# automl/CARL

Measured on AMD Instinct MI355X. Metric: env-steps/sec (whole node) at 65k parallel contexts, 1/2/4/8 MI355X, higher is better.
Workload: dtype f32

## Files before the change

### carl_amd/csrc/carl_amd.hip

```cpp
#include <hip/hip_runtime.h>

#include <cmath>
#include <cstdarg>
#include <cstdio>
#include <cstdlib>
#include <cstring>
#include <map>
#include <mutex>
#include <utility>

#include "../../include/carl_amd.h"
#include "classic_control.hip.h"
#include "context_kernels.hip.h"
#include "engine_kernels.hip.h"
#include "host_common.hpp"

namespace carl_host {

thread_local char g_err[512] = "";

int fail(int code, const char* fmt, ...) {
  va_list ap;
  va_start(ap, fmt);
  vsnprintf(g_err, sizeof g_err, fmt, ap);
// ... 124 lines not shown
}

}

namespace {

using carl_host::check_launch;
using carl_host::fail;
using carl_host::kInfo;
using carl_host::validate_batch;
using carl_host::with_classic_family;

int validate_io(const carl_batch_t* b, const carl_step_io_t* io, const char* who) {
  if (io == nullptr) return fail(CARL_ERR_INVALID_ARGUMENT, "%s: io is NULL", who);
  if (!io->action || !io->obs || !io->reward || !io->terminated || !io->truncated)
    return fail(CARL_ERR_INVALID_ARGUMENT, "%s: a required io pointer is NULL", who);
  const bool discrete = kInfo[b->family].action_is_discrete != 0;
  if (discrete && io->action_dtype != CARL_ACTION_I32 && io->action_dtype != CARL_ACTION_I64 &&
      io->action_dtype != CARL_ACTION_U8)
    return fail(CARL_ERR_INVALID_ARGUMENT, "%s: discrete family needs int32/int64 (carl_rollout: or uint8) actions", who);
  if (io->action_dtype == CARL_ACTION_U8 && (reinterpret_cast<uintptr_t>(io->action) & 3) != 0)
    return fail(CARL_ERR_INVALID_ARGUMENT, "%s: uint8 actions must be 4-byte aligned", who);
  const bool half = io->action_dtype == CARL_ACTION_F16 || io->action_dtype == CARL_ACTION_BF16;
  if (!discrete && io->action_dtype != CARL_ACTION_F32 && !half)
    return fail(CARL_ERR_INVALID_ARGUMENT, "%s: continuous family needs float32 (carl_rollout: or float16 / bfloat16) actions", who);
  if (half && (reinterpret_cast<uintptr_t>(io->action) & 7) != 0)
    return fail(CARL_ERR_INVALID_ARGUMENT, "%s: float16 / bfloat16 actions must be 8-byte aligned", who);
  if (io->row_pitch != 0 && io->row_pitch < b->n_lanes)
    return fail(CARL_ERR_INVALID_ARGUMENT, "%s: io.row_pitch %d < n_lanes %d (0 = dense rows)", who, io->row_pitch, b->n_lanes);
  return 0;
}

template <class Fam>
bool use_lds_ctx(const carl_batch_t* b) {
  const size_t bytes = (size_t)Fam::F * b->n_contexts * sizeof(float);
  return bytes <= 32 * 1024 && (int64_t)b->n_contexts * 8 <= (int64_t)b->n_lanes;
}

int row_pitch_of(const carl_batch_t* b, const carl_step_io_t* io) { return io->row_pitch > 0 ? io->row_pitch : b->n_lanes; }

struct RolloutPlan {
  int variant = CARL_ROLLOUT_STAGED;
  bool lean = false;
  bool unsupported = false;
  int ak = 0;
  bool plain = false, ldsctx = false, moves = false, fin = false, ar = false, deep = false;
  size_t lds_bytes = 0;
};

template <class Fam>
RolloutPlan plan_rollout(const carl_batch_t* b, const carl_step_io_t* io) {
  static_assert(carl::predraw_of<Fam>::value, "the staged kernels below are instantiated for predrawing families");
  RolloutPlan p;
  const int dt = io->action_dtype;
  p.ak = dt == CARL_ACTION_I64 ? 1 : dt == CARL_ACTION_U8 ? carl::kActU8 : dt == CARL_ACTION_F16 ? carl::kActF16
         : dt == CARL_ACTION_BF16 ? carl::kActBF16 : 0;
  const uintptr_t amask = p.ak == carl::kActU8 ? 3u : p.ak > carl::kActU8 ? 7u : 15u;
  if (b->flags & CARL_FLAG_ROLLOUT_DIRECT)
    p.variant = CARL_ROLLOUT_DIRECT_FLAG;
  else if (!carl_host::staged_rows(b, io, amask))
    p.variant = CARL_ROLLOUT_DIRECT_SHAPE;
  const bool keeps_context = b->selector == CARL_SEL_STATIC || b->selector == CARL_SEL_HOST;
  p.lean = p.variant == CARL_ROLLOUT_STAGED && keeps_context && b->fin_count == nullptr && io->final_obs == nullptr;
  p.unsupported = p.ak >= carl::kActU8 && !p.lean;
  if (p.variant != CARL_ROLLOUT_STAGED) return p;

  p.lds_bytes = carl::rollout_staged_lds_bytes<Fam>();
  const size_t table_bytes = (size_t)Fam::F * b->n_contexts * sizeof(float);
  const bool table_fits =
      use_lds_ctx<Fam>(b) && p.lds_bytes + table_bytes + carl::static_lds_bytes<Fam>() <= carl::kCuLdsBytes;
  if (p.lean) {
    p.plain = true;
    p.ar = carl::dense_done_of<Fam>::value && (b->flags & CARL_FLAG_AUTORESET);
    p.deep = p.ak == 0 && b->n_lanes < carl::deep_below_lanes_of<Fam>::value;
  } else if (carl::dense_done_of<Fam>::value && b->fin_count == nullptr) {
    p.plain = true;
    p.moves = !keeps_context;
    p.fin = io->final_obs != nullptr;
    p.ldsctx = p.moves && table_fits;
  } else {
    p.ldsctx = !keeps_context && table_fits;
  }
  if (p.ldsctx) p.lds_bytes += table_bytes;
  return p;
}

using staged_kern_t = void (*)(carl_batch_t, carl_step_io_t, int);

template <class Fam>
staged_kern_t staged_kernel(const RolloutPlan& p) {
#define CARL_STAGED(AK, PLAIN, LDSCTX, MOVES, FIN, AR, DEEP)                                                         \
  if (p.ak == AK && p.plain == PLAIN && p.ldsctx == LDSCTX && p.moves == MOVES && p.fin == FIN && p.ar == AR &&    \
      p.deep == DEEP)                                                                                              \
    return carl::rollout_staged_kernel<Fam, AK, bool(PLAIN), bool(LDSCTX), bool(MOVES), bool(FIN), bool(AR), bool(DEEP)>;
#define CARL_STAGED_01(...) CARL_STAGED(0, __VA_ARGS__) CARL_STAGED(1, __VA_ARGS__)
  constexpr bool dense = carl::dense_done_of<Fam>::value, deep = carl::deep_below_lanes_of<Fam>::value > 0;
  CARL_STAGED_01(    0,     0,    0,  0, 0,   0)
  CARL_STAGED_01(    0,     1,    0,  0, 0,   0)
  CARL_STAGED_01(    1,     0,    0,  0, 0,   0)
  if constexpr (std::is_same_v<typename Fam::Action, int>) {
    CARL_STAGED(carl::kActU8, 1, 0, 0, 0, 0, 0)
  } else {
    CARL_STAGED(carl::kActF16, 1, 0, 0, 0, 0, 0)
    CARL_STAGED(carl::kActBF16, 1, 0, 0, 0, 0, 0)
  }
  if constexpr (deep) CARL_STAGED(0, 1, 0, 0, 0, 0, 1)
  if constexpr (dense) {
    CARL_STAGED_01(  1,     0,    0,  0, 1,   0)
    CARL_STAGED(carl::kActU8, 1, 0, 0, 0, 1, 0)
    if constexpr (deep) CARL_STAGED(0, 1, 0, 0, 0, 1, 1)
    CARL_STAGED_01(  1,     0,    0,  1, 0,   0)
    CARL_STAGED_01(  1,     0,    1,  0, 0,   0)
    CARL_STAGED_01(  1,     0,    1,  1, 0,   0)
    CARL_STAGED_01(  1,     1,    1,  0, 0,   0)
    CARL_STAGED_01(  1,     1,    1,  1, 0,   0)
  }
#undef CARL_STAGED_01
#undef CARL_STAGED
  return nullptr;
}

int pick_block(int n, bool lds) { return (lds || n > 256 * 1024) ? 256 : 64; }

template <class Fam>
int step_block(const carl_batch_t* b) { return pick_block(b->n_lanes, use_lds_ctx<Fam>(b)); }

template <class Fam>
int launch_reset(const carl_batch_t* b, const uint8_t* mask, const int32_t* idx, const int32_t* count, float* obs,
                 hipStream_t s) {
  if (b->n_lanes == 0) return 0;
  const bool lds = use_lds_ctx<Fam>(b);
  const int block = 256;
  int grid = (b->n_lanes + block - 1) / block;
  if (grid > 4096) grid = 4096;
  if (lds) {
    const size_t sh = (size_t)Fam::F * b->n_contexts * sizeof(float);
    hipLaunchKernelGGL((carl::reset_kernel<Fam, true>), dim3(grid), dim3(block), sh, s, *b, mask, idx, count, obs);
  } else {
    hipLaunchKernelGGL((carl::reset_kernel<Fam, false>), dim3(grid), dim3(block), 0, s, *b, mask, idx, count, obs);
  }
  return check_launch("carl_reset");
}

template <class Fam>
int launch_step(const carl_batch_t* b, const carl_step_io_t* io, int n_steps, hipStream_t s) {
  if (b->n_lanes == 0 || n_steps == 0) return 0;
  const bool rollout = n_steps >= 0;
  const RolloutPlan plan = plan_rollout<Fam>(b, io);
  if (plan.unsupported || (!rollout && plan.ak >= carl::kActU8))
    return fail(CARL_ERR_UNSUPPORTED,
                "uint8 / float16 / bfloat16 actions: carl_rollout in its lean staged configuration only (row pitch %% 16 == 0, "
                "static / host selector, no finished-episode log, no final_obs); pass int32 / int64 / float32 actions");
  carl_step_io_t io_resolved = *io;
  io_resolved.row_pitch = row_pitch_of(b, io);
  if (rollout && plan.variant == CARL_ROLLOUT_STAGED) {
    const staged_kern_t kern = staged_kernel<Fam>(plan);
    if (kern == nullptr) return fail(CARL_ERR_UNSUPPORTED, "carl_rollout: no staged kernel for this configuration");
    if (int e = carl_host::ensure_dynamic_lds(reinterpret_cast<const void*>(kern), plan.lds_bytes, "carl_rollout")) return e;
    const int grid = (b->n_lanes + carl::kRolloutLanes - 1) / carl::kRolloutLanes;
    hipLaunchKernelGGL(kern, dim3(grid), dim3(carl::kStagedThreads), plan.lds_bytes, s, *b, io_resolved, n_steps);
    return check_launch("carl_rollout");
  }
  const bool lds = use_lds_ctx<Fam>(b), a64 = io->action_dtype == CARL_ACTION_I64;
  const int block = rollout ? carl::kRolloutThreads : step_block<Fam>(b);
  const int lanes_per_block = rollout ? carl::kRolloutLanes : block;
  const dim3 g((b->n_lanes + lanes_per_block - 1) / lanes_per_block), t(block);
// ... 254 lines not shown
```

### carl_amd/csrc/classic_control.hip.h

```cpp
#pragma once

#include <type_traits>

#include "carl_device.hip.h"
#include "fast_math.hip.h"
#include "host_common.hpp"

namespace carl {

constexpr float kPi = 3.14159265358979323846f;

struct NoAux {};

struct CartPole {
  static constexpr int S = 4, D = 4, F = 8;
  using Action = int;
  using Aux = NoAux;
  enum { GRAVITY, MASSCART, MASSPOLE, LENGTH, FORCE_MAG, TAU, INIT_LO, INIT_HI };
  static constexpr bool kNeedsStepNoise = false;
  static constexpr bool kPredraw = true;
  static constexpr int kDeepBelowLanes = 65536;
  static constexpr bool kDenseDone = true;

  struct Params {
    float gravity, masspole, length, force_mag, tau, inv_total_mass, polemass_length;
    float init_lo, init_hi;
  };

  template <class Ctx>
  __device__ static __forceinline__ Params load(const Ctx& ctx, int c, int flags) {
    Params p;
    p.gravity = ctx.get(GRAVITY, c);
    p.masspole = ctx.get(MASSPOLE, c);
    p.length = ctx.get(LENGTH, c);
    p.force_mag = ctx.get(FORCE_MAG, c);
    p.tau = ctx.get(TAU, c);
    float total_mass;
    if (flags & CARL_FLAG_CARTPOLE_RECOMPUTE) {
      total_mass = p.masspole + ctx.get(MASSCART, c);
      p.polemass_length = p.masspole * p.length;
    } else {
      total_mass = 0.1f + 1.0f;
      p.polemass_length = 0.1f * 0.5f;
    }
    p.inv_total_mass = 1.0f / total_mass;
    p.init_lo = ctx.get(INIT_LO, c);
    p.init_hi = ctx.get(INIT_HI, c);
    return p;
  }

  __device__ static __forceinline__ void prepare(const float (&)[S], Aux&) {}

  __device__ static __forceinline__ bool out_of_bounds(float x, float theta) {
    const float x_thr = 2.4f;
    const float th_thr = (float)(12.0 * 2.0 * 3.14159265358979323846 / 360.0);
    return (x < -x_thr) | (x > x_thr) | (theta < -th_thr) | (theta > th_thr);
  }

  __device__ static __forceinline__ bool step(const Params& p, float (&s)[S], Aux&, int action, float ,
                                              int elapsed, float& reward) {
#pragma clang fp contract(off)
    const float x = s[0], x_dot = s[1], theta = s[2], theta_dot = s[3];
    const bool was_terminated = (elapsed > 0) && out_of_bounds(x, theta);
    const float force = (action == 1) ? p.force_mag : -p.force_mag;
    float sintheta, costheta;
    sincos_fast_smallarg(theta, sintheta, costheta);
    const float temp = __fmaf_rn(p.polemass_length * (theta_dot * theta_dot), sintheta, force) * p.inv_total_mass;
    const float num = __fmaf_rn(-costheta, temp, p.gravity * sintheta);
    const float den = p.length * __fmaf_rn(-(p.masspole * (costheta * costheta)), p.inv_total_mass, 4.0f / 3.0f);
    const float thetaacc = div_fast(num, den);
    const float xacc = __fmaf_rn(-((p.polemass_length * thetaacc) * costheta), p.inv_total_mass, temp);
    s[0] = __fmaf_rn(p.tau, x_dot, x);
    s[1] = __fmaf_rn(p.tau, xacc, x_dot);
    s[2] = __fmaf_rn(p.tau, theta_dot, theta);
    s[3] = __fmaf_rn(p.tau, thetaacc, theta_dot);
    const bool terminated = out_of_bounds(s[0], s[2]);
    reward = (terminated && was_terminated) ? 0.0f : 1.0f;
    return terminated;
  }

  __device__ static __forceinline__ void observe(const float (&s)[S], const Aux&, float (&o)[D]) {
#pragma unroll
    for (int i = 0; i < 4; ++i) o[i] = s[i];
  }

  __device__ static __forceinline__ void reset(const Params& p, const u32x4& w, float (&s)[S]) {
    const float lo = p.init_lo, hi = p.init_hi;
    s[0] = uniform_between(lo, hi, w.x);
    s[1] = uniform_between(lo, hi, w.y);
    s[2] = uniform_between(lo, hi, w.z);
    s[3] = uniform_between(lo, hi, w.w);
  }
};

struct Pendulum {
  static constexpr int S = 2, D = 3, F = 7;
  using Action = float;
  enum { GRAVITY_DEAD, DT, G, M, L, INIT_ANGLE_MAX, INIT_VEL_MAX };
  static constexpr bool kNeedsStepNoise = false;
  static constexpr bool kPredraw = true;
  static constexpr int kDeepBelowLanes = 32768;

  struct Params {
    float c_sin;
    float c_u;
    float dt;
    float init_angle_max, init_vel_max;
  };
  struct Aux {
    float sn, cs;
  };

  template <class Ctx>
  __device__ static __forceinline__ Params load(const Ctx& ctx, int c, int) {
    const float g = ctx.get(G, c), m = ctx.get(M, c), l = ctx.get(L, c);
    return Params{3.0f * g / (2.0f * l), 3.0f / (m * (l * l)), ctx.get(DT, c), ctx.get(INIT_ANGLE_MAX, c),
                  ctx.get(INIT_VEL_MAX, c)};
  }

  __device__ static __forceinline__ void prepare(const float (&s)[S], Aux& a) { sincos_fast_pk(s[0], a.sn, a.cs); }

  __device__ static __forceinline__ bool step(const Params& p, float (&s)[S], Aux& aux, float action,
                                              float , int , float& reward) {
#pragma clang fp contract(off)
    const float max_speed = 8.0f, max_torque = 2.0f;
    const float th = s[0], thdot = s[1];
    const float u = fminf(fmaxf(action, -max_torque), max_torque);
    const float inv_two_pi = 1.0f / (2.0f * kPi);
    const float two_pi_hi = 0x1.921fb6p+2f, two_pi_lo = -0x1.777a5cp-23f;
    const float turns = rintf(th * inv_two_pi);
    const float a0 = fabsf(__fmaf_rn(-turns, two_pi_lo, __fmaf_rn(-turns, two_pi_hi, th)));
    const float an = (a0 > kPi) ? (two_pi_hi - a0) + two_pi_lo : a0;
    const float costs = __fmaf_rn(an, an, __fmaf_rn(0.1f, thdot * thdot, 0.001f * (u * u)));
    float newthdot = __fmaf_rn(__fmaf_rn(p.c_sin, aux.sn, p.c_u * u), p.dt, thdot);
    newthdot = fminf(fmaxf(newthdot, -max_speed), max_speed);
    s[0] = __fmaf_rn(newthdot, p.dt, th);
    s[1] = newthdot;
    sincos_fast_pk(s[0], aux.sn, aux.cs);
    reward = -costs;
    return false;
  }

  __device__ static __forceinline__ void observe(const float (&s)[S], const Aux& a, float (&o)[D]) {
    o[0] = a.cs;
    o[1] = a.sn;
    o[2] = s[1];
  }

  __device__ static __forceinline__ void reset(const Params& p, const u32x4& w, float (&s)[S]) {
    s[0] = uniform_between(0.0f, p.init_angle_max, w.x);
    s[1] = uniform_between(0.0f, p.init_vel_max, w.y);
  }
};

#include "sincos_table.inc"
__device__ const double kSinCosTab[2 * CARL_SINCOS_TAB_N] = {CARL_SINCOS_TAB_VALUES};

struct SinCosTab {
  typedef double vd2 __attribute__((ext_vector_type(2)));
  __device__ static __forceinline__ vd2* lds() {
    __shared__ vd2 tab[CARL_SINCOS_TAB_N];
    return tab;
  }
  __device__ static __forceinline__ void stage() {
    vd2* t = lds();
    const vd2* g = reinterpret_cast<const vd2*>(kSinCosTab);
    for (int i = threadIdx.x; i < CARL_SINCOS_TAB_N; i += blockDim.x) t[i] = g[i];
  }
  struct Pending {
    vd2 ea, eb;
    double ra, rb;
  };
  __device__ static __forceinline__ Pending lookup2(double xa, double xb) {
    const vd2* t = lds();
    const double inv = CARL_SINCOS_TAB_INV_STEP, hi = CARL_SINCOS_TAB_STEP_HI;
// ... 388 lines not shown
```

### carl_amd/csrc/engine_kernels.hip.h

```cpp
#pragma once

#include <type_traits>

#include "carl_device.hip.h"


namespace carl {

template <bool LDS>
using ctx_t = std::conditional_t<LDS, LdsCtx, GlobalCtx>;

template <class Fam, class = void>
struct has_tables : std::false_type {};
template <class Fam>
struct has_tables<Fam, std::void_t<decltype(Fam::kUsesSinCosTab)>> : std::bool_constant<Fam::kUsesSinCosTab> {};

template <class Fam>
__device__ __forceinline__ void stage_family_tables() {
  if constexpr (has_tables<Fam>::value) {
    Fam::stage_tables();
    __syncthreads();
  }
}

// ... 208 lines not shown
  }
}

template <class Fam>
__device__ __forceinline__ void finish_plain(const carl_batch_t& b, uint64_t glane, bool done, float (&o)[Fam::D],
                                             LaneRegs<Fam>& r) {
  u32x4 w = r.next_w;
  if (ballot(done && !r.next_ok) != 0ull) {
    const u32x4 wi = lane_words(b.seed, glane, r.episode, kSubInit);
    w = select_words(r.next_ok, w, wi);
  }
  float ns[Fam::S], no[Fam::D];
  typename Fam::Aux na;
  Fam::reset(r.p, w, ns);
  Fam::prepare(ns, na);
  Fam::observe(ns, na, no);
  const bool rs = done && (b.flags & CARL_FLAG_AUTORESET) != 0;
  r.fin_return = done ? r.ep_return : r.fin_return;
  r.fin_length = done ? r.elapsed : r.fin_length;
  r.n_new_episodes += done ? 1 : 0;
#pragma unroll
  for (int j = 0; j < Fam::S; ++j) r.s[j] = rs ? ns[j] : r.s[j];
#pragma unroll
  for (int d = 0; d < Fam::D; ++d) o[d] = rs ? no[d] : o[d];
  r.aux = select_words(rs, na, r.aux);
  r.elapsed = rs ? 0 : r.elapsed;
  r.ep_return = rs ? 0.0f : r.ep_return;
  r.episode += rs ? 1u : 0u;
  r.n_new_calls += rs ? 1 : 0;
  r.next_ok = r.next_ok && !rs;
  __builtin_amdgcn_s_waitcnt(0xC07F);
}

template <class Fam, class = void>
struct deep_action_prefetch_of : std::false_type {};
template <class Fam>
struct deep_action_prefetch_of<Fam, std::void_t<decltype(Fam::kDeepActionPrefetch)>> : std::bool_constant<Fam::kDeepActionPrefetch> {};

template <class Fam, class = void>
struct deep_below_lanes_of : std::integral_constant<int, 0> {};
template <class Fam>
struct deep_below_lanes_of<Fam, std::void_t<decltype(Fam::kDeepBelowLanes)>> : std::integral_constant<int, Fam::kDeepBelowLanes> {};

template <class Fam, class = void>
struct dense_done_of : std::false_type {};
template <class Fam>
struct dense_done_of<Fam, std::void_t<decltype(Fam::kDenseDone)>> : std::bool_constant<Fam::kDenseDone> {};

template <class Fam>
struct DenseNext {
  unsigned long long ok_mask;
  float s[Fam::S];
  typename Fam::Aux aux;
  int cidx;
  typename Fam::Params p;
};

template <class Fam, class Ctx, bool MOVES>
__device__ __forceinline__ void dense_draw(const carl_batch_t& b, const Ctx& ctx, uint64_t glane,
                                           const LaneRegs<Fam>& r, unsigned long long lanes, DenseNext<Fam>& nx) {
  int cn = r.cidx;
  typename Fam::Params pn = r.p;
  if constexpr (MOVES) {
    cn = select_context(b, r.cidx, glane, r.episode);
    if (ballot(cn != r.cidx) != 0ull) {
      typename Fam::Params q = Fam::load(ctx, cn, b.flags);
      settle(q);
      pn = select_words(cn != r.cidx, q, r.p);
    }
  }
  const u32x4 w = lane_words(b.seed, glane, r.episode, kSubInit);
  float fresh[Fam::S];
  typename Fam::Aux fa;
  Fam::reset(pn, w, fresh);
  Fam::prepare(fresh, fa);
  const bool mine = ((lanes >> lane_id()) & 1ull) != 0ull;
#pragma unroll
  for (int j = 0; j < Fam::S; ++j) nx.s[j] = mine ? fresh[j] : nx.s[j];
  nx.aux = select_words(mine, fa, nx.aux);
  if constexpr (MOVES) {
    nx.cidx = mine ? cn : nx.cidx;
    nx.p = select_words(mine, pn, nx.p);
  }
}

template <class Fam, class Ctx, bool MOVES, bool FINAL, bool AR, bool ENTRY, class Sink>
__device__ __forceinline__ void step_dense(const carl_batch_t& b, const Ctx& ctx, const Sink& cur, int max_steps_eff,
                                           bool autoreset_in, uint64_t glane, typename Fam::Action action,
                                           LaneRegs<Fam>& r, DenseNext<Fam>& nx) {
  static_assert(!Fam::kNeedsStepNoise, "dense done handling: families without per-step noise");
  const bool autoreset = AR || autoreset_in;
  float reward;
  const bool terminated = Fam::step(r.p, r.s, r.aux, action, 0.0f, (AR && !ENTRY) ? 0 : r.elapsed, reward);
  r.elapsed += 1;
  const bool truncated = r.elapsed >= max_steps_eff;
  r.ep_return += reward;
  cur.put_reward(reward);
  cur.put_flags(terminated, truncated);
  const bool done = terminated | truncated;
  const unsigned long long dm = ballot(done);
  const unsigned long long again = dm & ~nx.ok_mask;
  if (__builtin_expect(again != 0ull, 0)) dense_draw<Fam, Ctx, MOVES>(b, ctx, glane, r, again, nx);
  const bool rs = done && autoreset;
  if constexpr (FINAL) {
    if (rs && r.valid) {
      float fo[Fam::D];
      Fam::observe(r.s, r.aux, fo);
      store_obs<Fam::D>(cur.final_obs_ptr(), 0, fo);
    }
  }
  r.fin_return = done ? r.ep_return : r.fin_return;
  r.fin_length = done ? r.elapsed : r.fin_length;
  r.n_new_episodes += done ? 1 : 0;
#pragma unroll
  for (int j = 0; j < Fam::S; ++j) r.s[j] = rs ? nx.s[j] : r.s[j];
  r.aux = select_words(rs, nx.aux, r.aux);
  if constexpr (MOVES) {
    r.cidx = rs ? nx.cidx : r.cidx;
    r.p = select_words(rs, nx.p, r.p);
  }
  r.elapsed = rs ? 0 : r.elapsed;
  r.ep_return = rs ? 0.0f : r.ep_return;
  r.episode += rs ? 1u : 0u;
  if constexpr (!AR) r.n_new_calls += rs ? 1 : 0;
  nx.ok_mask &= autoreset ? ~dm : ~0ull;
  float o[Fam::D];
  Fam::observe(r.s, r.aux, o);
  cur.put_obs(o);
}

template <class Fam, class Ctx, bool ALL_ACTIVE = false, class Sink = Cursors<Fam>, bool PLAIN = false>
__device__ __forceinline__ void step_lane(const carl_batch_t& b, const Ctx& ctx, const Sink& cur,
                                          int max_steps, bool active_in, int lane, uint64_t glane,
                                          typename Fam::Action action, LaneRegs<Fam>& r) {
  const bool active = ALL_ACTIVE || active_in;
  bool done = false;
  bool te = false, tr = false;
  float o[Fam::D];
  if (active) {
    float noise = 0.0f;
    if constexpr (Fam::kNeedsStepNoise) noise = Fam::step_noise(r.p, b, glane, r.episode - 1u, r.elapsed);
    float reward;
    const bool terminated = Fam::step(r.p, r.s, r.aux, action, noise, r.elapsed, reward);
    r.elapsed += 1;
    const bool truncated = (max_steps > 0) && (r.elapsed >= max_steps);
    r.ep_return += reward;
    Fam::observe(r.s, r.aux, o);
    cur.put_reward(reward);
    if constexpr (!Sink::kLazyFlags) cur.put_flags(terminated, truncated);
    te = terminated;
    tr = truncated;
    done = terminated | truncated;
  }
  if (__builtin_expect(ballot(done) != 0ull, 0)) {
    if constexpr (Sink::kLazyFlags) {
      if (active) cur.put_flags(te, tr);
    }
    if constexpr (PLAIN)
      finish_plain<Fam>(b, glane, done, o, r);
    else
      finish_episodes<Fam, Ctx, Sink::kLazyFlags && predraw_of<Fam>::value>(b, ctx, done, lane, glane,
                                                                            cur.final_obs_ptr(), o, r);
  }
  if (active) cur.put_obs(o);
}

// ... 116 lines not shown
  Action tmp[CHUNK][4];
#pragma unroll
  for (int u = 0; u < CHUNK; ++u) {
    const AStore* row = act + (size_t)(t0 + u) * n;
    const bool row_ok = t0 + u < n_steps;
#pragma unroll
    for (int k = 0; k < 4; ++k) tmp[u][k] = (row_ok && first + k < (int)n) ? (Action)row[first + k] : Action{};
  }
#pragma unroll
  for (int u = 0; u < CHUNK; ++u) {
    Action* dst = buf + u * kRolloutLanes + 4 * l;
#pragma unroll
    for (int k = 0; k < 4; ++k) dst[k] = tmp[u][k];
  }
}

template <class Fam, bool LDS, bool A64>
__global__ void __launch_bounds__(kRolloutThreads) rollout_kernel(const carl_batch_t b, const carl_step_io_t io,
                                                                  const int n_steps) {
  extern __shared__ float lds_dyn[];
  stage_family_tables<Fam>();
  using AStore = action_store_t<Fam, A64>;
  using Action = typename Fam::Action;
  Action* act_buf = reinterpret_cast<Action*>(lds_dyn);
  float* lds_ctx = lds_dyn + rollout_action_lds_bytes() / sizeof(float);
  const ctx_t<LDS> ctx = make_ctx<LDS, Fam::F>(b, lds_ctx);
  const bool loader = threadIdx.x >= kRolloutLanes;
  const int lane_base = blockIdx.x * kRolloutLanes;
  const int lane = lane_base + (loader ? 0 : (int)threadIdx.x);
  const bool active = !loader && lane < b.n_lanes;
  const uint64_t glane = (uint64_t)(b.lane_offset + lane);
  const size_t n = (size_t)io.row_pitch;
  const int max_steps = b.max_episode_steps;
  const AStore* act = static_cast<const AStore*>(io.action);
  LaneRegs<Fam> r{};
  Cursors<Fam> cur = make_cursors<Fam>(io, active ? lane : 0);
  if (loader)
    stage_actions<AStore, Action>(act_buf, act, n, lane_base, 0, n_steps);
  else if (active) {
    load_lane<Fam>(b, ctx, lane, r);
    if (!r.episode_valid) {
      r.episode = b.episode[lane];
      r.episode_valid = true;
      settle(r.episode);
    }
  }
  __syncthreads();
  int buf = 0;
  for (int t0 = 0; t0 < n_steps; t0 += kActChunk, buf ^= 1) {
    if (loader) {
      if (t0 + kActChunk < n_steps)
        stage_actions<AStore, Action>(act_buf + (buf ^ 1) * kActChunk * kRolloutLanes, act, n, lane_base,
                                      t0 + kActChunk, n_steps);
    } else {
      const Action* my = act_buf + buf * kActChunk * kRolloutLanes + threadIdx.x;
      const int steps = min(kActChunk, n_steps - t0);
      Action a_next = my[0];
      settle(a_next);
      if (lane_base + kRolloutLanes <= b.n_lanes) {
        for (int u = 0; u < steps; ++u) {
          const Action a = a_next;
          a_next = my[min(u + 1, kActChunk - 1) * kRolloutLanes];
          step_lane<Fam, ctx_t<LDS>, true>(b, ctx, cur, max_steps, true, lane, glane, a, r);
          cur.advance(n);
        }
      } else {
        for (int u = 0; u < steps; ++u) {
          const Action a = a_next;
          a_next = my[min(u + 1, kActChunk - 1) * kRolloutLanes];
          step_lane<Fam>(b, ctx, cur, max_steps, active, lane, glane, a, r);
          cur.advance(n);
        }
      }
    }
    __syncthreads();
  }
  if (active) store_lane<Fam>(b, ctx, lane, r);
}

constexpr int kStageChunk = 8;
constexpr int kStorers = 3;
constexpr int kStagedThreads = kRolloutLanes + (1 + kStorers) * kWave;

template <class Fam, int CHUNK = kStageChunk>
__host__ __device__ constexpr size_t rollout_staged_lds_bytes() {
  return (size_t)2 * CHUNK * (LdsSink<Fam>::kStepBytes + kRolloutLanes * sizeof(float));
}

template <class AStore, class Action, int CHUNK, bool DEEP = false>
struct ActionPipe {
  static_assert(CHUNK == 8 || CHUNK == 4, "the in-flight chunk is held in eight (four) named register groups");
  static constexpr bool kSame = std::is_same_v<AStore, Action>;
  typedef float vf4 __attribute__((ext_vector_type(4)));
  typedef int vi4 __attribute__((ext_vector_type(4)));
  using V = std::conditional_t<std::is_same_v<Action, float>, vf4, vi4>;
  struct Wide {
    vi4 lo, hi;
  };
  static constexpr bool kU8 = std::is_same_v<AStore, unsigned char>;
  static constexpr bool kF16 = std::is_same_v<AStore, f16_bits>, kBF16 = std::is_same_v<AStore, bf16_bits>;
  typedef unsigned int vu2 __attribute__((ext_vector_type(2)));
  using R = std::conditional_t<kSame, V, std::conditional_t<kU8, unsigned int, std::conditional_t<kF16 || kBF16, vu2, Wide>>>;
  static constexpr bool kNarrow = kU8 || kF16 || kBF16;
  using LdsElem = std::conditional_t<kU8, unsigned char, std::conditional_t<kF16 || kBF16, unsigned short, Action>>;
  using LdsRow = std::conditional_t<kNarrow, R, V>;
  __device__ static __forceinline__ Action widen(LdsElem e) {
    if constexpr (kU8) {
      return (Action)e;
    } else if constexpr (kF16) {
      return (Action)__builtin_bit_cast(_Float16, e);
    } else if constexpr (kBF16) {
      return __uint_as_float((unsigned int)e << 16);
    } else {
      return e;
    }
  }
  R a0, a1, a2, a3, a4, a5, a6, a7;
  int t0;

  __device__ static __forceinline__ R load_row(const AStore* __restrict__ p) {
#define CARL_LD(q) __builtin_nontemporal_load(q)
    if constexpr (kSame) {
      return CARL_LD(reinterpret_cast<const V*>(p));
    } else if constexpr (kU8) {
      return CARL_LD(reinterpret_cast<const unsigned int*>(p));
    } else if constexpr (kF16 || kBF16) {
      return CARL_LD(reinterpret_cast<const vu2*>(p));
    } else {
      const vi4* q = reinterpret_cast<const vi4*>(p);
      return Wide{CARL_LD(q), CARL_LD(q + 1)};
    }
#undef CARL_LD
  }
  __device__ static __forceinline__ LdsRow narrow(const R& r) {
    if constexpr (kSame || kNarrow) {
      return r;
    } else {
      return V{r.lo.x, r.lo.z, r.hi.x, r.hi.z};
    }
  }

  bool fast;

  __device__ __forceinline__ void issue(const AStore* __restrict__ act, size_t n, int cols, int lane_base, int l, int t0_,
                                        int n_steps) {
    t0 = t0_;
    fast = t0 + CHUNK <= n_steps;
    if constexpr (DEEP) {
      const int lane4 = min(lane_base + 4 * l, cols - 4);
      const int last = n_steps - 1;
      a0 = load_row(act + (size_t)min(t0, last) * n + lane4);
      a1 = load_row(act + (size_t)min(t0 + 1, last) * n + lane4);
      a2 = load_row(act + (size_t)min(t0 + 2, last) * n + lane4);
      a3 = load_row(act + (size_t)min(t0 + 3, last) * n + lane4);
      if constexpr (CHUNK == 8) {
        a4 = load_row(act + (size_t)min(t0 + 4, last) * n + lane4);
        a5 = load_row(act + (size_t)min(t0 + 5, last) * n + lane4);
        a6 = load_row(act + (size_t)min(t0 + 6, last) * n + lane4);
        a7 = load_row(act + (size_t)min(t0 + 7, last) * n + lane4);
      }
      return;
    }
    if (!fast) return;
    const int lane4 = min(lane_base + 4 * l, cols - 4);
    const AStore* row = act + (size_t)t0 * n;
    a0 = load_row(row + lane4);
    row += n;
    a1 = load_row(row + lane4);
    row += n;
// ... 12 lines not shown
    }
  }
  __device__ __forceinline__ void commit(LdsElem* buf, const AStore* __restrict__ act, size_t n, int cols, int lane_base, int l,
                                         int n_steps) const {
    LdsRow* dst = reinterpret_cast<LdsRow*>(buf + 4 * l);
    constexpr int row = kRolloutLanes / 4;
    if (fast || DEEP) {
      dst[0] = narrow(a0);
      dst[row] = narrow(a1);
      dst[2 * row] = narrow(a2);
      dst[3 * row] = narrow(a3);
      if constexpr (CHUNK == 8) {
        dst[4 * row] = narrow(a4);
        dst[5 * row] = narrow(a5);
        dst[6 * row] = narrow(a6);
        dst[7 * row] = narrow(a7);
      }
      return;
    }
    const AStore* src = act + (size_t)t0 * n + min(lane_base + 4 * l, cols - 4);
#pragma unroll 1
    for (int u = 0; u < CHUNK && t0 + u < n_steps; ++u) dst[u * row] = narrow(load_row(src + (size_t)u * n));
  }
};

template <class Fam>
__device__ __forceinline__ void drain_records(char* buf, const carl_step_io_t& io, size_t n, int cols, int lane_base, int l,
                                              int which, int t0, int steps) {
  using SK = LdsSink<Fam>;
  const int valid = min(kRolloutLanes, cols - lane_base);
  typedef float vf4 __attribute__((ext_vector_type(4)));
  auto put = [](char* dst, const char* src) {
    const vf4 v = *reinterpret_cast<const vf4*>(src);
    __builtin_nontemporal_store(v, reinterpret_cast<vf4*>(dst));
  };
  for (int u = which; u < steps; u += kStorers) {
    char* rec = buf + (size_t)u * SK::kStepBytes;
    const size_t row = (size_t)(t0 + u) * n + lane_base;
    char* g_obs = reinterpret_cast<char*>(io.obs + row * Fam::D);
    char* fl = rec + SK::kFlagOff + 16 * l;
    const int fl_lane = 16 * (l & 15);
    uint8_t* fl_dst = (l < 16) ? io.terminated + row + fl_lane : io.truncated + row + fl_lane;
    if (valid == kRolloutLanes) {
#pragma unroll
      for (int off = 0; off < SK::kObsBytes; off += 1024) put(g_obs + off + 16 * l, rec + off + 16 * l);
      put(reinterpret_cast<char*>(io.reward + row) + 16 * l, rec + SK::kObsBytes + 16 * l);
      if (l < 32) put(reinterpret_cast<char*>(fl_dst), fl);
    } else {
#pragma unroll
      for (int off = 0; off < SK::kObsBytes; off += 1024)
        if (off + 16 * l < valid * Fam::D * 4) put(g_obs + off + 16 * l, rec + off + 16 * l);
      if (16 * l < valid * 4) put(reinterpret_cast<char*>(io.reward + row) + 16 * l, rec + SK::kObsBytes + 16 * l);
      if (l < 32 && fl_lane < valid) put(reinterpret_cast<char*>(fl_dst), fl);
    }
    if (l < 32) *reinterpret_cast<vf4*>(fl) = vf4{0.0f, 0.0f, 0.0f, 0.0f};
  }
}

template <class Fam, int CHUNK>
__device__ __forceinline__ void zero_flag_rows(char* out_buf, int l, int which) {
  using SK = LdsSink<Fam>;
  typedef float vf4 __attribute__((ext_vector_type(4)));
  if (l < 32)
    for (int u = which; u < 2 * CHUNK; u += kStorers)
      *reinterpret_cast<vf4*>(out_buf + (size_t)u * SK::kStepBytes + SK::kFlagOff + 16 * l) = vf4{0.0f, 0.0f, 0.0f, 0.0f};
}

template <class Fam, class Ctx>
__device__ __forceinline__ void load_staged_lane(const carl_batch_t& b, const Ctx& ctx, int lane, bool active,
                                                 LaneRegs<Fam>& r) {
  const int src = min(lane, b.n_lanes - 1);
  load_lane<Fam>(b, ctx, src, r);
  if (!r.episode_valid) {
    r.episode = b.episode[src];
    r.episode_valid = true;
    settle(r.episode);
  }
  r.valid = active;
}

template <class Fam, int A64, bool PLAIN, bool LDSCTX, bool MOVES, bool FINAL, bool AR, int CHUNK, bool DEEPALL = false>
__device__ __forceinline__ void rollout_staged_body(const carl_batch_t& b, const carl_step_io_t& io, const int n_steps,
                                                    const int wg, float* lds_dyn) {
  constexpr int kStageChunk = CHUNK;
  stage_family_tables<Fam>();
  using AStore = action_store_t<Fam, A64>;
  using Action = typename Fam::Action;
  using SK = LdsSink<Fam>;
  constexpr bool kDeep = !std::is_same_v<AStore, long long> &&
                         (DEEPALL || (deep_action_prefetch_of<Fam>::value && !std::is_same_v<AStore, Action>));
  using Pipe = ActionPipe<AStore, Action, kStageChunk, kDeep>;
  using LdsAct = typename Pipe::LdsElem;
  LdsAct* act_buf = reinterpret_cast<LdsAct*>(lds_dyn);
  char* out_buf = reinterpret_cast<char*>(lds_dyn) + (size_t)2 * kStageChunk * kRolloutLanes * sizeof(float);
  float* ctx_lds = reinterpret_cast<float*>(out_buf + (size_t)2 * kStageChunk * SK::kStepBytes);
  const ctx_t<LDSCTX> ctx = make_ctx<LDSCTX, Fam::F>(b, ctx_lds);
  const int wave = __builtin_amdgcn_readfirstlane((int)(threadIdx.x / kWave));
  const int storer = wave - (kRolloutLanes / kWave + 1);
  const bool compute = wave < kRolloutLanes / kWave;
  const bool loader = wave == kRolloutLanes / kWave;
  const int hl = threadIdx.x % kWave;
  const int lane_base = wg * kRolloutLanes;
  const int lane = lane_base + (compute ? (int)threadIdx.x : 0);
  const bool active = compute && lane < b.n_lanes;
  const uint64_t glane = (uint64_t)(b.lane_offset + lane);
  const size_t n = (size_t)io.row_pitch;
  const int n_cols = (b.n_lanes + 15) & ~15;
  const int max_steps = b.max_episode_steps;
  const AStore* act = static_cast<const AStore*>(io.action);
  constexpr int kBufActs = kStageChunk * kRolloutLanes;
  LaneRegs<Fam> r{};
  Pipe pipe;
  [[maybe_unused]] Pipe pipe_b;
  float* const final_base = (io.final_obs != nullptr && active) ? io.final_obs + (size_t)lane * Fam::D : nullptr;
  if (!compute && !loader) zero_flag_rows<Fam, CHUNK>(out_buf, hl, storer);
  if (loader) {
    pipe.issue(act, n, n_cols, lane_base, hl, 0, n_steps);
    pipe.commit(act_buf, act, n, n_cols, lane_base, hl, n_steps);
    pipe.issue(act, n, n_cols, lane_base, hl, kStageChunk, n_steps);
    if constexpr (kDeep) pipe_b.issue(act, n, n_cols, lane_base, hl, 2 * kStageChunk, n_steps);
  } else if (compute) {
    load_staged_lane<Fam>(b, ctx, lane, active, r);
  }
  __syncthreads();
  auto run_role = [&](auto role_tag) -> int {
  constexpr int ROLE = decltype(role_tag)::value;
  if constexpr (ROLE == 1 && kDeep) {
    int lbuf = 0;
    for (int t0 = 0;;) {
      pipe.commit(act_buf + (lbuf ^ 1) * kBufActs, act, n, n_cols, lane_base, hl, n_steps);
      pipe.issue(act, n, n_cols, lane_base, hl, t0 + 3 * kStageChunk, n_steps);
      __syncthreads();
      lbuf ^= 1;
      if (t0 + kStageChunk >= n_steps) break;
      pipe_b.commit(act_buf + (lbuf ^ 1) * kBufActs, act, n, n_cols, lane_base, hl, n_steps);
      pipe_b.issue(act, n, n_cols, lane_base, hl, t0 + 4 * kStageChunk, n_steps);
      __syncthreads();
      lbuf ^= 1;
      t0 += 2 * kStageChunk;
      if (t0 >= n_steps) break;
    }
    return lbuf;
  }
  int buf = 0;
  [[maybe_unused]] DenseNext<Fam> nx{};
  [[maybe_unused]] const bool autoreset = (b.flags & CARL_FLAG_AUTORESET) != 0;
  [[maybe_unused]] const int max_steps_eff = max_steps > 0 ? max_steps : 0x7fffffff;
  for (int t0 = 0; t0 < n_steps; t0 += kStageChunk, buf ^= 1) {
    const int steps = min(kStageChunk, n_steps - t0);
    if constexpr (ROLE == 0) {
      const LdsAct* my = act_buf + buf * kBufActs + threadIdx.x;
      char* rec = out_buf + (size_t)buf * kStageChunk * SK::kStepBytes;
      if constexpr (PLAIN && dense_done_of<Fam>::value) {
        if (nx.ok_mask != ~0ull) {
          dense_draw<Fam, ctx_t<LDSCTX>, MOVES>(b, ctx, glane, r, ~nx.ok_mask, nx);
          nx.ok_mask = ~0ull;
        }
        Action acts[kStageChunk];
#pragma unroll
        for (int u = 0; u < kStageChunk; ++u) acts[u] = Pipe::widen(my[u * kRolloutLanes]);
        if (steps == kStageChunk) {
#pragma unroll
          for (int u = 0; u < kStageChunk; ++u) {
            const SK sink{rec + (size_t)u * SK::kStepBytes, FINAL ? final_base : nullptr, n * Fam::D, t0 + u,
                          (int)threadIdx.x};
            if (u == 0)
              step_dense<Fam, ctx_t<LDSCTX>, MOVES, FINAL, AR, true, SK>(b, ctx, sink, max_steps_eff, autoreset, glane,
                                                                         acts[u], r, nx);
            else
              step_dense<Fam, ctx_t<LDSCTX>, MOVES, FINAL, AR, false, SK>(b, ctx, sink, max_steps_eff, autoreset, glane,
                                                                          acts[u], r, nx);
          }
        } else {
#pragma unroll 1
          for (int u = 0; u < steps; ++u) {
            const SK sink{rec + (size_t)u * SK::kStepBytes, FINAL ? final_base : nullptr, n * Fam::D, t0 + u,
                          (int)threadIdx.x};
            Action a = acts[0];
#pragma unroll
            for (int k = 1; k < kStageChunk; ++k) a = (u == k) ? acts[k] : a;
            step_dense<Fam, ctx_t<LDSCTX>, MOVES, FINAL, AR, true, SK>(b, ctx, sink, max_steps_eff, autoreset, glane, a, r,
                                                                       nx);
          }
        }
        if constexpr (AR) r.n_new_calls = r.n_new_episodes;
      }
      if constexpr (!(PLAIN && dense_done_of<Fam>::value)) {
      if constexpr (predraw_of<Fam>::value) predraw<Fam>(b, glane, r);
      if (PLAIN && steps == kStageChunk) {
        Action acts[kStageChunk];
#pragma unroll
        for (int u = 0; u < kStageChunk; ++u) acts[u] = Pipe::widen(my[u * kRolloutLanes]);
#pragma unroll
        for (int u = 0; u < kStageChunk; ++u) {
          const SK sink{rec + (size_t)u * SK::kStepBytes, final_base, n * Fam::D, t0 + u, (int)threadIdx.x};
          step_lane<Fam, ctx_t<LDSCTX>, true, SK, PLAIN>(b, ctx, sink, max_steps, true, lane, glane, acts[u], r);
        }
      } else {
      Action a_next = Pipe::widen(my[0]);
      settle(a_next);
      for (int u = 0; u < steps; ++u) {
        const Action a = a_next;
        a_next = Pipe::widen(my[min(u + 1, kStageChunk - 1) * kRolloutLanes]);
        const SK sink{rec + (size_t)u * SK::kStepBytes, final_base, n * Fam::D, t0 + u, (int)threadIdx.x};
        step_lane<Fam, ctx_t<LDSCTX>, true, SK, PLAIN>(b, ctx, sink, max_steps, true, lane, glane, a, r);
      }
      }
      }
    } else if constexpr (ROLE == 1) {
      pipe.commit(act_buf + (buf ^ 1) * kBufActs, act, n, n_cols, lane_base, hl, n_steps);
      pipe.issue(act, n, n_cols, lane_base, hl, t0 + 2 * kStageChunk, n_steps);
    } else if (t0 > 0) {
      drain_records<Fam>(out_buf + (size_t)(buf ^ 1) * kStageChunk * SK::kStepBytes, io, n, n_cols, lane_base, hl, storer,
                         t0 - kStageChunk, kStageChunk);
    }
    __syncthreads();
  }
  return buf;
  };
  const int buf = compute ? run_role(std::integral_constant<int, 0>{})
                          : loader ? run_role(std::integral_constant<int, 1>{}) : run_role(std::integral_constant<int, 2>{});
  if (compute) {
    if (active) store_lane<Fam>(b, ctx, lane, r);
  } else if (!loader) {
    const int last_t0 = ((n_steps - 1) / kStageChunk) * kStageChunk;
    drain_records<Fam>(out_buf + (size_t)(buf ^ 1) * kStageChunk * SK::kStepBytes, io, n, n_cols, lane_base, hl, storer,
                       last_t0, n_steps - last_t0);
  }
}

template <class Fam, int A64, bool PLAIN = false, bool LDSCTX = false, bool MOVES = false, bool FINAL = false,
          bool AR = false, bool DEEPALL = false>
__global__ void __launch_bounds__(kStagedThreads) rollout_staged_kernel(const carl_batch_t b, const carl_step_io_t io,
                                                                        const int n_steps) {
  extern __shared__ float lds_dyn[];
  rollout_staged_body<Fam, A64, PLAIN, LDSCTX, MOVES, FINAL, AR, kStageChunk, DEEPALL>(b, io, n_steps, (int)blockIdx.x,
                                                                                        lds_dyn);
}

constexpr int kPairChunk = 4;

template <class FamA, class FamB>
__host__ __device__ constexpr size_t rollout_pair_lds_bytes() {
  constexpr size_t a = rollout_staged_lds_bytes<FamA, kPairChunk>(), b = rollout_staged_lds_bytes<FamB, kPairChunk>();
  return a > b ? a : b;
}

template <class FamA, class FamB, bool ARA, bool ARB>
__global__ void __launch_bounds__(kStagedThreads) __attribute__((amdgpu_waves_per_eu(4)))
rollout_staged_pair_kernel(const carl_batch_t ba, const carl_step_io_t ioa, const carl_batch_t bb, const carl_step_io_t iob,
                           const int n_steps, const int grid_a) {
  extern __shared__ float lds_dyn[];
  if ((int)blockIdx.x < grid_a)
    rollout_staged_body<FamA, false, true, false, false, false, ARA && dense_done_of<FamA>::value, kPairChunk>(
        ba, ioa, n_steps, (int)blockIdx.x, lds_dyn);
  else
    rollout_staged_body<FamB, false, true, false, false, false, ARB && dense_done_of<FamB>::value, kPairChunk>(
        bb, iob, n_steps, (int)blockIdx.x - grid_a, lds_dyn);
}

}
```

Measured before the change: 205.1 billion.

## Precompute next-episode reset states on helper waves via LDS draw-ahead ring

Adds an LDS ring that the loader and storer waves fill with the next episode's initial state for each lane, computed from the per-lane episode counter the compute waves publish each chunk. In the dense autoreset path, compute waves pick up the precomputed state instead of running the RNG and reset inline, and fall back to dense_draw when the tag does not match. This moves reset RNG work off the critical compute waves into otherwise idle helper waves, at the cost of extra LDS, and applies only to CartPole, the one family with reset_words.

```diff
diff --git a/carl_amd/csrc/carl_amd.hip b/carl_amd/csrc/carl_amd.hip
--- a/carl_amd/csrc/carl_amd.hip
+++ b/carl_amd/csrc/carl_amd.hip
@@ -230,6 +230,8 @@
     p.ldsctx = !keeps_context && table_fits;
   }
   if (p.ldsctx) p.lds_bytes += table_bytes;
+  if (carl::staged_draw_ahead<Fam>(p.plain, p.ldsctx, p.moves, p.fin, p.ar, carl::kStageChunk, p.deep))
+    p.lds_bytes = carl::rollout_staged_lds_bytes<Fam>(true);
   return p;
 }
 
diff --git a/carl_amd/csrc/classic_control.hip.h b/carl_amd/csrc/classic_control.hip.h
--- a/carl_amd/csrc/classic_control.hip.h
+++ b/carl_amd/csrc/classic_control.hip.h
@@ -91,6 +91,17 @@
     s[2] = uniform_between(lo, hi, w.z);
     s[3] = uniform_between(lo, hi, w.w);
   }
+  static constexpr int kResetWords = 2;
+  __device__ static __forceinline__ void reset_words(const Params& p, float (&w)[kResetWords]) {
+    w[0] = p.init_lo;
+    w[1] = p.init_hi;
+  }
+  __device__ static __forceinline__ Params reset_params(const float (&w)[kResetWords]) {
+    Params p{};
+    p.init_lo = w[0];
+    p.init_hi = w[1];
+    return p;
+  }
 };
 
 struct Pendulum {
diff --git a/carl_amd/csrc/engine_kernels.hip.h b/carl_amd/csrc/engine_kernels.hip.h
--- a/carl_amd/csrc/engine_kernels.hip.h
+++ b/carl_amd/csrc/engine_kernels.hip.h
@@ -314,6 +314,75 @@
     nx.cidx = mine ? cn : nx.cidx;
     nx.p = select_words(mine, pn, nx.p);
   }
+}
+
+template <class Fam, class = void>
+struct reset_words_of : std::integral_constant<int, 0> {};
+template <class Fam>
+struct reset_words_of<Fam, std::void_t<decltype(Fam::kResetWords)>> : std::integral_constant<int, Fam::kResetWords> {};
+
+constexpr bool kDrawAheadFullSize = true;
+
+template <class Fam>
+struct DrawRing {
+  static constexpr int kLanes = 256;
+  static constexpr int kWords = reset_words_of<Fam>::value;
+  static constexpr size_t kSlotBytes = (size_t)kLanes * (Fam::S + 1) * 4;
+  static constexpr size_t kBytes = (size_t)kLanes * (2 + kWords) * 4 + 2 * kSlotBytes;
+  char* base;
+  __device__ __forceinline__ uint32_t* episodes(int parity) const {
+    return reinterpret_cast<uint32_t*>(base) + parity * kLanes;
+  }
+  __device__ __forceinline__ float* reset_words() const { return reinterpret_cast<float*>(base) + 2 * kLanes; }
+  __device__ __forceinline__ float* slot_state(uint32_t episode) const {
+    return reinterpret_cast<float*>(base + (size_t)kLanes * (2 + kWords) * 4 + (episode & 1u) * kSlotBytes);
+  }
+  __device__ __forceinline__ uint32_t* slot_tag(uint32_t episode) const {
+    return reinterpret_cast<uint32_t*>(slot_state(episode) + kLanes * Fam::S);
+  }
+  __device__ __forceinline__ void open(int tid, const typename Fam::Params& p, uint32_t episode) const {
+    float w[kWords];
+    Fam::reset_words(p, w);
+#pragma unroll
+    for (int k = 0; k < kWords; ++k) reset_words()[k * kLanes + tid] = w[k];
+    episodes(1)[tid] = episode;
+  }
+  __device__ __forceinline__ void invalidate(int tid) const {
+    slot_tag(0u)[tid] = 1u;
+    slot_tag(1u)[tid] = 0u;
+  }
+  __device__ __forceinline__ void produce(int tid, int parity, uint64_t seed, uint64_t glane,
+                                          const float (&rw)[kWords > 0 ? kWords : 1]) const {
+    const uint32_t e = episodes(parity)[tid] + 1u;
+    const u32x4 w = lane_words(seed, glane, e, kSubInit);
+    float fresh[Fam::S];
+    Fam::reset(Fam::reset_params(rw), w, fresh);
+    store_obs<Fam::S>(slot_state(e), (size_t)tid, fresh);
+    slot_tag(e)[tid] = e;
+  }
+};
+
+template <class Fam, class Ctx>
+__device__ __forceinline__ void dense_pickup(const carl_batch_t& b, const Ctx& ctx, uint64_t glane, const DrawRing<Fam>& ring,
+                                             int tid, const LaneRegs<Fam>& r, unsigned long long lanes, DenseNext<Fam>& nx) {
+  const uint32_t tag = ring.slot_tag(r.episode)[tid];
+  const float* src = ring.slot_state(r.episode) + (size_t)tid * Fam::S;
+  float fresh[Fam::S];
+  if constexpr (Fam::S == 4) {
+    const float4 v = *reinterpret_cast<const float4*>(src);
+    fresh[0] = v.x, fresh[1] = v.y, fresh[2] = v.z, fresh[3] = v.w;
+  } else {
+#pragma unroll
+    for (int j = 0; j < Fam::S; ++j) fresh[j] = src[j];
+  }
+  typename Fam::Aux fa;
+  Fam::prepare(fresh, fa);
+  const bool mine = ((lanes >> lane_id()) & 1ull) != 0ull;
+#pragma unroll
+  for (int j = 0; j < Fam::S; ++j) nx.s[j] = mine ? fresh[j] : nx.s[j];
+  nx.aux = select_words(mine, fa, nx.aux);
+  const unsigned long long missed = lanes & ballot(tag != r.episode);
+  if (__builtin_expect(missed != 0ull, 0)) dense_draw<Fam, Ctx, false>(b, ctx, glane, r, missed, nx);
 }
 
 template <class Fam, class Ctx, bool MOVES, bool FINAL, bool AR, bool ENTRY, class Sink>
@@ -596,9 +665,17 @@
 constexpr int kStorers = 3;
 constexpr int kStagedThreads = kRolloutLanes + (1 + kStorers) * kWave;
 
+template <class Fam>
+__host__ __device__ constexpr bool staged_draw_ahead(bool plain, bool ldsctx, bool moves, bool fin, bool ar, int chunk,
+                                                     bool deepall) {
+  return reset_words_of<Fam>::value > 0 && dense_done_of<Fam>::value && plain && ar && !ldsctx && !moves && !fin &&
+         chunk == kStageChunk && (deepall || kDrawAheadFullSize);
+}
+
 template <class Fam, int CHUNK = kStageChunk>
-__host__ __device__ constexpr size_t rollout_staged_lds_bytes() {
-  return (size_t)2 * CHUNK * (LdsSink<Fam>::kStepBytes + kRolloutLanes * sizeof(float));
+__host__ __device__ constexpr size_t rollout_staged_lds_bytes(bool draw_ahead = false) {
+  return (size_t)2 * CHUNK * (LdsSink<Fam>::kStepBytes + kRolloutLanes * sizeof(float)) +
+         (draw_ahead ? DrawRing<Fam>::kBytes : 0);
 }
 
 template <class AStore, class Action, int CHUNK, bool DEEP = false>
@@ -777,6 +854,7 @@
 template <class Fam, int A64, bool PLAIN, bool LDSCTX, bool MOVES, bool FINAL, bool AR, int CHUNK, bool DEEPALL = false>
 __device__ __forceinline__ void rollout_staged_body(const carl_batch_t& b, const carl_step_io_t& io, const int n_steps,
                                                     const int wg, float* lds_dyn) {
+  constexpr bool kAhead = staged_draw_ahead<Fam>(PLAIN, LDSCTX, MOVES, FINAL, AR, CHUNK, DEEPALL);
   constexpr int kStageChunk = CHUNK;
   stage_family_tables<Fam>();
   using AStore = action_store_t<Fam, A64>;
@@ -809,6 +887,14 @@
   [[maybe_unused]] Pipe pipe_b;
   float* const final_base = (io.final_obs != nullptr && active) ? io.final_obs + (size_t)lane * Fam::D : nullptr;
   if (!compute && !loader) zero_flag_rows<Fam, CHUNK>(out_buf, hl, storer);
+  [[maybe_unused]] const DrawRing<Fam> ring{reinterpret_cast<char*>(ctx_lds)};
+  [[maybe_unused]] const int htid = (int)threadIdx.x - kRolloutLanes;
+  [[maybe_unused]] const uint64_t hglane = (uint64_t)(b.lane_offset + lane_base + htid);
+  if constexpr (kAhead) {
+    static_assert(DrawRing<Fam>::kLanes == kRolloutLanes && 1 + kStorers == kRolloutLanes / kWave,
+                  "one helper wave per compute wave");
+    if (!compute) ring.invalidate(htid);
+  }
   if (loader) {
     pipe.issue(act, n, n_cols, lane_base, hl, 0, n_steps);
     pipe.commit(act_buf, act, n, n_cols, lane_base, hl, n_steps);
@@ -816,20 +902,28 @@
     if constexpr (kDeep) pipe_b.issue(act, n, n_cols, lane_base, hl, 2 * kStageChunk, n_steps);
   } else if (compute) {
     load_staged_lane<Fam>(b, ctx, lane, active, r);
+    if constexpr (kAhead) ring.open((int)threadIdx.x, r.p, r.episode);
   }
   __syncthreads();
   auto run_role = [&](auto role_tag) -> int {
   constexpr int ROLE = decltype(role_tag)::value;
+  [[maybe_unused]] float rw[DrawRing<Fam>::kWords > 0 ? DrawRing<Fam>::kWords : 1];
+  if constexpr (kAhead && ROLE != 0) {
+#pragma unroll
+    for (int k = 0; k < DrawRing<Fam>::kWords; ++k) rw[k] = ring.reset_words()[k * kRolloutLanes + htid];
+  }
   if constexpr (ROLE == 1 && kDeep) {
     int lbuf = 0;
     for (int t0 = 0;;) {
       pipe.commit(act_buf + (lbuf ^ 1) * kBufActs, act, n, n_cols, lane_base, hl, n_steps);
       pipe.issue(act, n, n_cols, lane_base, hl, t0 + 3 * kStageChunk, n_steps);
+      if constexpr (kAhead) ring.produce(htid, lbuf ^ 1, b.seed, hglane, rw);
       __syncthreads();
       lbuf ^= 1;
       if (t0 + kStageChunk >= n_steps) break;
       pipe_b.commit(act_buf + (lbuf ^ 1) * kBufActs, act, n, n_cols, lane_base, hl, n_steps);
       pipe_b.issue(act, n, n_cols, lane_base, hl, t0 + 4 * kStageChunk, n_steps);
+      if constexpr (kAhead) ring.produce(htid, lbuf ^ 1, b.seed, hglane, rw);
       __syncthreads();
       lbuf ^= 1;
       t0 += 2 * kStageChunk;
@@ -848,7 +942,10 @@
       char* rec = out_buf + (size_t)buf * kStageChunk * SK::kStepBytes;
       if constexpr (PLAIN && dense_done_of<Fam>::value) {
         if (nx.ok_mask != ~0ull) {
-          dense_draw<Fam, ctx_t<LDSCTX>, MOVES>(b, ctx, glane, r, ~nx.ok_mask, nx);
+          if constexpr (kAhead)
+            dense_pickup<Fam, ctx_t<LDSCTX>>(b, ctx, glane, ring, (int)threadIdx.x, r, ~nx.ok_mask, nx);
+          else
+            dense_draw<Fam, ctx_t<LDSCTX>, MOVES>(b, ctx, glane, r, ~nx.ok_mask, nx);
           nx.ok_mask = ~0ull;
         }
         Action acts[kStageChunk];
@@ -879,6 +976,7 @@
           }
         }
         if constexpr (AR) r.n_new_calls = r.n_new_episodes;
+        if constexpr (kAhead) ring.episodes(buf)[threadIdx.x] = r.episode;
       }
       if constexpr (!(PLAIN && dense_done_of<Fam>::value)) {
       if constexpr (predraw_of<Fam>::value) predraw<Fam>(b, glane, r);
@@ -909,6 +1007,7 @@
       drain_records<Fam>(out_buf + (size_t)(buf ^ 1) * kStageChunk * SK::kStepBytes, io, n, n_cols, lane_base, hl, storer,
                          t0 - kStageChunk, kStageChunk);
     }
+    if constexpr (kAhead && ROLE != 0) ring.produce(htid, buf ^ 1, b.seed, hglane, rw);
     __syncthreads();
   }
   return buf;
```

After: 201.2 billion. 0.981x the previous value.
